# coin-or/Ipopt

Hardware: AMD Instinct MI355X
Metric: KKT factor+solve GFLOP/s (1 numeric LDL^T factorisation + 2 solves per Ipopt iteration) (higher is better)
Workload: dtype f64; 1 GPU; synth_1e6; kkt_dim=1000000, triplet_nnz=20143342, nnz_L=230755000, ordering=nested dissection + minimum-degree leaves (own), supernodes=50052, tree_levels=110, maxfront=3260, num_neg=400000

## Files before the change

ipopt_amd/csrc/device_view.hip.inc:

```
constexpr int FLAG_STRIDE = 32;

typedef double v2d __attribute__((ext_vector_type(2)));
struct DevView {
    const int* sn_colptr; const int* sn_rowptr; const int* sn_rows; const int* rel;
    const int* child_ptr; const int* child_idx; const int* sn_owner; const int* sn_parent; const int* col_owner;
    const long long* panel_off; const long long* cb_off; const long long* minv_off;
    const int* acolptr; const int* apos; const int* arow; const int* acol;
    const int* dup_ptr; const int* dup_src;
    const int* rslot_ptr; const int* rslot_idx; const int* rslot_col; int rslot_len;
    const int* level_sn;
    const FrontMeta* fmeta;
    const int* relinv;
    const GroupLink* gtab;
    const int* tile_tab;
    const ChildMeta* cmeta;
    const int* perm;
    const double* tvals;
    double* aval;
    double* scale;
    double* scale2;
    double* arv;
    unsigned long long* rowmax;
    double* L;
    double* cb;
// ... 18 lines not shown
    unsigned long long* strace;
    const int* chwg_f; const int* chwg_b; const int* chwait; int* sflag_t; int* sflag_dot; double* dpart; v2d* ytag; v2d* xtag;
    int xcd_affine;
    int* apfail;
    int* tcnt;
    double* isg; int* hasis;
    const int* lc_ptr; const LeafLink* lc_link;
    int* sflag_s;
    v2d* cbt; const long long* cbt_off;
    int* sflag_p;
    int* sflag_b; int* sflag_d; int* sepoch;
    int* zpiv;
    int n, nnz_a, nsn, rank;
    int fastpiv;
    double fastu;
    int asm_pull;
    int norestore;
    unsigned long long* dbg;
};

template <int CTRL>
__device__ __forceinline__ double dpp_f64(double x)
{
    int lo = __double2loint(x), hi = __double2hiint(x);
    lo = __builtin_amdgcn_update_dpp(lo, lo, CTRL, 0xF, 0xF, false);
    hi = __builtin_amdgcn_update_dpp(hi, hi, CTRL, 0xF, 0xF, false);
    return __hiloint2double(hi, lo);
}
__device__ __forceinline__ double readlane_f64(double x, int l)
{
// ... 37 lines not shown
```

ipopt_amd/csrc/kernels_big.hip.inc:

```
typedef double v4f64 __attribute__((ext_vector_type(4)));
typedef double double2a __attribute__((ext_vector_type(2), aligned(8)));

__device__ __forceinline__ void big_assemble_column(const DevView& V, const FrontMeta& M, const int fc, const int top_mode)
{
    const int s = M.s, c0 = M.c0, k = M.k, r0 = M.r0, m = M.m; (void)s; (void)c0; (void)r0; (void)k;
    const int lane = threadIdx.x & 63;
    const bool active = fc < m && !(M.asmcut && fc >= M.asmcut);
    double* col = nullptr;
    const bool from_arena = top_mode && V.arena && V.arena_off[s] >= 0;
    const bool skip_owned = top_mode && V.arena;
    if (active) {
        const double* Ar = from_arena ? V.arena + V.arena_off[s] + (size_t)fc * (m - 1) - ((size_t)fc * (fc - 1)) / 2 : nullptr;
        if (fc < k) col = V.L + M.panel_off + (size_t)fc * M.ldp;
        else        col = V.cb + M.cb_off + (size_t)(fc - k) * M.ldt - k;
        if (M.alias) {
            if (from_arena) for (int i = fc + lane; i < m; i += 64) col[i] += Ar[i];
        } else if (V.asm_pull) {
            const double* Cc[4]; const int* Iv[4]; int nc = 0;
            for (int cp = M.ch0; cp < M.ch1 && nc < 4; ++cp) {
                const ChildMeta Cm = V.cmeta[cp];
                if (Cm.aliased || (skip_owned && Cm.owner >= 0) || fc < Cm.rlo || fc > Cm.rhi) continue;
                const int lo = V.relinv[Cm.inv + fc];
                if (lo < 0) continue;
                Cc[nc] = V.cb + Cm.cb_off + (size_t)lo * Cm.ldt; Iv[nc] = V.relinv + Cm.inv; ++nc;
// ... 705 lines not shown
            acc[0][1] = __builtin_amdgcn_mfma_f64_16x16x4f64(a0[u], b1[u], acc[0][1], 0, 0, 0);
            acc[1][0] = __builtin_amdgcn_mfma_f64_16x16x4f64(a1[u], b0[u], acc[1][0], 0, 0, 0);
            acc[1][1] = __builtin_amdgcn_mfma_f64_16x16x4f64(a1[u], b1[u], acc[1][1], 0, 0, 0);
        }
#pragma unroll
    for (int r = 0; r < 2; ++r)
#pragma unroll
        for (int q = 0; q < 2; ++q)
#pragma unroll
            for (int g = 0; g < 4; ++g) {
                const int c = cc0 + r * 16 + l4 + 4 * g, i = i0 + q * 16 + l15;
                if (i < mu && c < climit && i >= c) T[i + (size_t)c * M.ldt] = tv[r][q][g] - acc[r][q][g];
            }
}

__global__ __launch_bounds__(256) void k_big_diag_trsm(DevView V, int list_off, int nrb)
{
    extern __shared__ __attribute__((aligned(16))) char smem_raw[];
    const FrontMeta M = V.fmeta[list_off + blockIdx.x];
    const int role = blockIdx.y;
    const int epoch = V.sepoch[2];
#ifdef MI355X_PIVSTAT
    const bool tprobe = gridDim.x == 1 && threadIdx.x == 0;
    if (tprobe && role == 0) g_dt[0] = wall_clock64();
    if (tprobe && role == 1) g_dt[6] = wall_clock64();
#endif
    if (role == 0) { big_diag_body<4, 256>(V, M, smem_raw, &V.sflag_d[M.s], epoch, nullptr, nullptr, FrontMeta(), 0, 0, V.norestore ? &V.sflag_p[M.s] : nullptr); return; }
    const int tid = threadIdx.x;
    const int s = M.s, k = M.k, m = M.m;
    if (role > nrb) {
        const int t = role - 1 - nrb;
        const int mu = m - k, nt = (mu + 63) >> 6;
        if (M.grem <= 0 || t >= nt * ((M.grem + 63) >> 6)) return;
        if (tid == 0) {
            int spins = 0;
            while (__hip_atomic_load(&V.tcnt[s], __ATOMIC_RELAXED, __HIP_MEMORY_SCOPE_AGENT) < nt) { __builtin_amdgcn_s_sleep(16);
                if (++spins > (1 << 24)) { V.qstat[1] = 1; break; } }
        }
        __syncthreads();
        __builtin_amdgcn_fence(__ATOMIC_ACQUIRE, "agent");
        narrow_tile64(V, M, t);
        return;
// ... 261 lines not shown
        schur_tile_body<64, 64, 256, SCHURQ_LD>(V, M, i0, cc0, mu, 0, 0, As, Bs);
        __syncthreads();
    }
}

__global__ __launch_bounds__(256, 4) void k_big_schur64(DevView V, int list_off, int mode)
{
    int tx = blockIdx.x, fy = blockIdx.y;
    if (V.xcd_affine) xcd_affine(tx, fy);
    const FrontMeta M = V.fmeta[list_off + fy];
    schur64_tile(V, M, tx, mode);
}


constexpr size_t GRP_DB_BYTES = (size_t)64 * 65 * sizeof(double);
__device__ __forceinline__ void grp_fused_body(const DevView& V, const int list_off, const int staged_arg, const int rbw, const int role0)
{
    const int staged = staged_arg;
    extern __shared__ __attribute__((aligned(16))) char smem_raw[];
    const int tid = threadIdx.x, lane = tid & 63, wave = tid >> 6;
    const int l15 = lane & 15, l4 = lane >> 4;
    const FrontMeta M = V.fmeta[list_off + blockIdx.x];
    const int g = M.gpos + 1, role = (int)blockIdx.y + role0;
    const int tail = M.m - M.k;
    int myq = -1, eb0 = 0, nsub = 1;
    if (role < 4) { if (role >= g) return; myq = role; }
    else { eb0 = 64 * rbw * (role - 4); if (eb0 >= tail) return; nsub = min(rbw, (tail - eb0 + 63) >> 6); }
    const int epoch = V.sepoch[2];
#define GSTAMP(i) do { if (V.dbg && blockIdx.x == 0 && role < 4 && tid == 0) V.dbg[32 + 8 * role + (i)] = wall_clock64(); } while (0)
    GSTAMP(0);
// ... 169 lines not shown
    }
    }
    if (myq < 0) return;
    {
        double* Pq = V.L + Gq.panel_off;
        const size_t ldq = (size_t)Gq.ldp;
        const int i = tid & 63, cq = tid >> 6, kq = Gq.k;
        if (!V.norestore) {
#pragma unroll
        for (int e = 0; e < 16; ++e) { const int c = cq + 4 * e; if (i < kq && c < kq && i >= c) Pq[i + (size_t)c * ldq] = Db[i + c * ldb]; }
        }
        FrontMeta Mq = M;
        Mq.s = Gq.s; Mq.c0 = Gq.c0; Mq.k = Gq.k; Mq.m = Gq.m; Mq.panel_off = Gq.panel_off; Mq.ldp = Gq.ldp; Mq.wb = Gq.wb; Mq.minv_off = Gq.minv_off;
        Mq.selfasm = 0; Mq.aq0 = Gq.aq0; Mq.aq1 = Gq.aq1; Mq.bigidx = Gq.bigidx;
        __syncthreads();
        big_diag_body<4, 256, true>(V, Mq, smem_raw, &V.sflag_d[Gq.s], epoch, tsp, crit_Lr, crit_Mp, crit_ibase, myrows, (V.norestore && staged) ? &V.sflag_p[Gq.s] : nullptr);
        if (tsp && tid == 0) { for (int q = 0; q < 28; ++q) V.dbg[64 + q] = tsp[q]; }
        GSTAMP(7);
    }
#undef GSTAMP
}
__global__ __launch_bounds__(256) void k_grp_fused(DevView V, int list_off, int staged, int rbw, int role0) { grp_fused_body(V, list_off, staged, rbw, role0); }
```

ipopt_amd/csrc/kernels_fronts.hip.inc:

```
template <int TS>
__device__ __forceinline__ void publish_col(double* buf, const double (&t)[TS][TS], const int row0, const int jl)
{
#pragma unroll
    for (int b = 0; b < TS; ++b)
        if (jl == b) {
#pragma unroll
            for (int a = 0; a < TS; ++a) { double v = t[a][b]; asm volatile("" : "+v"(v)); buf[row0 + a] = v; }
        }
}

#ifdef MI355X_PIVSTAT
__device__ unsigned long long g_fstat[32];
__device__ unsigned long long g_dt[16], g_dtacc[16];
__device__ unsigned long long g_pivstat[16];
#ifdef MI355X_PIVSTAT_COUNT
#define PIVSTAT(i) do { if (threadIdx.x == 0) atomicAdd(&g_pivstat[i], 1ull); } while (0)
#else
#define PIVSTAT(i) do { } while (0)
#endif
#else
#define PIVSTAT(i) do { } while (0)
#endif

__device__ __forceinline__ double fast_rcp(double d)
// ... 571 lines not shown
                    const int cc = 16 * tc + l15;
#pragma unroll
                    for (int g = 0; g < 4; ++g) { const int rr = 16 * ti + l4 + 4 * g; if (rr < k && cc < k) Lb[rr + cc * ld] -= acc[g]; }
                }
        }
        if (pub) asm volatile("s_waitcnt vmcnt(0)" ::: "memory");
        __syncthreads();
        if (ts) { if (b == 0) ts[18] = clock64(); if (b == 1) ts[21] = clock64(); if (b == 2) ts[24] = clock64(); }
        if (wave == 0) PSTAMP(7);
    }
#undef PSTAMP
    nneg += neg;
    return true;
}

template <int J> __device__ __forceinline__ void fast16_step(double (&a)[16], double (&w)[16], double& rsave, const int l15)
{
    const double t = a[J];
    w[J] = t;
    const double d = bcast16<J>(t);
    const double ri = fast_rcp(d);
    rsave = (l15 == J) ? ri : rsave;
    const double l = t * ri;
    rank1_dpp16<J>(a, t, l);
    a[J] = l;
}
template <int J> __device__ __forceinline__ void fast16_inv(const double (&a)[16], double (&x)[4], const int l15, const int k)
{
    const double m = (l15 > J && l15 < k) ? -a[J] : 0.0;
    subst_dpp16<J>(x[0], m);
// ... 519 lines not shown
        kprev = k; mprev = m; rlp = rl0;
        K0 = K1; K1 = K2;
#pragma unroll
        for (int j = 0; j < 3; ++j) { pos0[j] = pos1[j]; val0[j] = val1[j]; }
        cn0 = cn1; rl0 = rl1;
    }
}

__device__ __forceinline__ void chain_signal(int* flag, const int epoch);
__device__ __forceinline__ void chain_signal_coh(int* flag, const int epoch);
__device__ __forceinline__ void st_coh(double* p, double v);
__device__ __forceinline__ void st_coh(int* p, int v);
__device__ __forceinline__ void st16_coh(double* p, double v0, double v1);
template <int NAP = 2> __device__ __forceinline__ void chain_wait(const int* flag, const int epoch, int* err);
__device__ __forceinline__ void trsm_store_l(const DevView& V, const FrontMeta& M, const double* Lr, const int ibase, const int rlim);
template <int TS, int NT, bool PRE = false>
__device__ __forceinline__ void big_diag_body(const DevView& V, const FrontMeta& M, char* smem_raw, int* flag = nullptr, const int epoch = 0, unsigned long long* ts = nullptr,
                                              const double* late_Lr = nullptr, const FrontMeta& late_M = FrontMeta(), const int late_ibase = 0, const int late_rows = 0, int* pflag = nullptr)
{
    constexpr int G = (NT == 1024) ? 32 : 16, MAXM = G * TS;
    const int tid = threadIdx.x;
    const int s = M.s, c0 = M.c0, k = M.k;
    const int ld = k | 1;
    double* Lb     = reinterpret_cast<double*>(smem_raw);
    double* colbuf = Lb + (size_t)ld * k;
    double* dinv_s = colbuf + 4 * MAXM; double* doff_s = dinv_s + k; double* cm0 = doff_s + k;
    int* ord = reinterpret_cast<int*>(cm0 + k); int* pt_s = ord + k;
    double* P = V.L + M.panel_off;
    const size_t ldp = (size_t)M.ldp;
    int nneg = 0, nzero = 0, ntwo = 0, nsmall = 0, chg = 0;
    DBGSTAMP(0);
// ... 19 lines not shown
#pragma unroll
                    for (int e = 0; e < 2; ++e) { const int q = M.aq0 + tid + e * NT; if (q < M.aq1) { apos_[e] = V.apos[q]; aval_[e] = V.aval[q]; na = e + 1; } }
                }
#pragma unroll
                for (int e = 0; e < 16; ++e) { const int c = cq + 4 * e; if (i < k && c < k && i >= c) { Lb[i + c * ld] = pv[e]; Lb[c + i * ld] = pv[e]; } }
                __syncthreads();
                if (M.selfasm) {
#pragma unroll
                    for (int e = 0; e < 2; ++e) if (e < na) { const int ii = apos_[e] % M.m, cc = apos_[e] / M.m; if (ii < k) { Lb[ii + cc * ld] += aval_[e]; if (ii != cc) Lb[cc + ii * ld] += aval_[e]; } }
                    for (int q = M.aq0 + tid + 2 * NT; q < M.aq1; q += NT) { const int pos = V.apos[q]; const int ii = pos % M.m, cc = pos / M.m; if (ii < k) { const double v = V.aval[q]; Lb[ii + cc * ld] += v; if (ii != cc) Lb[cc + ii * ld] += v; } }
                    __syncthreads();
                }
            }
            DBGT(1);
            if (ts) ts[8] = clock64();
            double cmx;
            {
                const int c = tid >> 2, part = tid & 3;
                double mx = 0.0;
                if (c < k) for (int r = part; r < k; r += 4) mx = fmax(mx, fabs(PRE ? Lb[max(r, c) + min(r, c) * ld] : Lb[r + c * ld]));
                mx = fmax(mx, dpp_f64<0xB1>(mx)); mx = fmax(mx, dpp_f64<0x4E>(mx));
                if (c < k && part == 0) mx = fmax(mx, V.cnorm[c0 + c]); else if (c >= k) mx = 0.0;
                cmx = wave_max_all(mx);
                if ((tid & 63) == 0) colbuf[tid >> 6] = cmx;
                __syncthreads();
                cmx = fmax(fmax(colbuf[0], colbuf[1]), fmax(colbuf[2], colbuf[3]));
            }
            const double zmax = fmax(V.small, ZERO_REL * cmx);
            const double gmax = 1.0 / fmax(fmax(V.pivtol, V.pivtol2), V.fastu);
            DBGT(2);
            if (ts) ts[9] = clock64();
            if (pflag) {
                const PubHook H{P, ldp, V.dinv + c0, V.isg + (size_t)M.bigidx * ISG_STRIDE, pflag, 8 * epoch};
                fast = ldlt_blocked_static(Lb, ld, k, Wp, dinv_s, Isb, shflag, zmax, gmax, nneg, V.dbg, ts, &H);
                if (!fast && tid == 0) __hip_atomic_store(pflag, 8 * epoch + 7, __ATOMIC_RELAXED, __HIP_MEMORY_SCOPE_AGENT);
            } else
            fast = ldlt_blocked_static(Lb, ld, k, Wp, dinv_s, Isb, shflag, zmax, gmax, nneg, V.dbg, ts);
            DBGT(3);
            if (ts) ts[10] = clock64();
            if (fast) {
                DBGSTAMP(1);
#pragma unroll
                for (int e = 0; e < 16; ++e) { const int c = cq + 4 * e; if (i < k && c < k) { const double v = (i > c) ? Lb[i + c * ld] : 0.0; if (flag) st_coh(&P[i + (size_t)c * ldp], v); else P[i + (size_t)c * ldp] = v; if (i <= c) Lb[i + c * ld] = 0.0; } }
                for (int j = tid; j < k; j += NT) { doff_s[j] = 0.0; pt_s[j] = 1; ord[j] = j; }
                {
                    double* Ig = V.isg + (size_t)M.bigidx * ISG_STRIDE;
                    const int nis = ((k + 15) >> 4) * 272;
                    if (flag) { for (int idx = tid; idx < nis; idx += NT) st_coh(&Ig[idx], Isb[idx]); }
                    else for (int idx = tid; idx < nis; idx += NT) Ig[idx] = Isb[idx];
                }
                if (tid == 0) atomicAdd(&V.qstat[3], 1);
                __syncthreads();
// ... 54 lines not shown
#endif
    invert_unit_lower<NT>(Lb, ld, k);
    DBGSTAMP(3);
#ifdef MI355X_PIVSTAT
    if (dprobe) g_dt[4] = wall_clock64();
#endif
    double* Mg = V.minv + M.minv_off;
    for (int idx = tid; idx < k * k; idx += NT) { const int i = idx % k, c = idx / k; Mg[idx] = (i > c) ? Lb[i + c * ld] : (i == c ? 1.0 : 0.0); }
    if (V.dbg && blockIdx.x == 0 && tid == 0) V.dbg[15] = (unsigned long long)k;
}

static size_t diag_lds_bytes(int kk, int maxm)
{
    return (size_t)((kk | 1) * kk + 4 * maxm + 3 * kk) * sizeof(double) + (size_t)(2 * kk + 2) * sizeof(int) + (size_t)(16 * 65 + 4 * 272) * sizeof(double) + 64;
}
template <int TS, int NT = 256>
__global__ __launch_bounds__(NT) void k_big_diag_reg(DevView V, int list_off)
{
    extern __shared__ __attribute__((aligned(16))) char smem_raw[];
    const FrontMeta M = V.fmeta[list_off + blockIdx.x];
    big_diag_body<TS, NT>(V, M, smem_raw);
}

__global__ void k_reduce_stats(const int4* fstat, const int* apfail, const int* owner, int nsn, int rank_filter, int* out)
{
    __shared__ int sh[4][256];
    int a = 0, b = 0, c = 0, d = 0;
    for (int s = blockIdx.x * 256 + threadIdx.x; s < nsn; s += gridDim.x * 256) {
        if (rank_filter >= -1 && owner[s] != rank_filter) continue;
        const int4 v = fstat[s]; a += v.x; b += v.y; c += v.z; d += v.w + apfail[s];
    }
    sh[0][threadIdx.x] = a; sh[1][threadIdx.x] = b; sh[2][threadIdx.x] = c; sh[3][threadIdx.x] = d;
    __syncthreads();
    for (int off = 128; off >= 1; off >>= 1) {
        if (threadIdx.x < off) for (int q = 0; q < 4; ++q) sh[q][threadIdx.x] += sh[q][threadIdx.x + off];
        __syncthreads();
// ... 13 lines not shown
```

ipopt_amd/csrc/numeric.hip:

```cpp
#include <hip/hip_runtime.h>
#include <rccl/rccl.h>
#include <dlfcn.h>
#include <cstdio>
#include <cstring>
#include <cmath>
#include <chrono>
#include <vector>
#include <thread>
#include <map>
#include <string>
#include <algorithm>
#include "numeric.h"
#include "launch_plan.h"
#include "env_knobs.h"
#include "matching_scaling.h"
#include "device_owner.h"
#include "lowrank_host.h"
#include "lbfgs_host.h"

namespace mi355x {

enum KernelKind { KK_GATHER_SCALE = 0, KK_FRONT_WAVE, KK_FRONT_LDS64, KK_FRONT_LDS128, KK_BIG_ASSEMBLE, KK_BIG_DIAG, KK_BIG_TRSM,
                  KK_BIG_SCHUR, KK_STATS, KK_SOLVE_PERM, KK_FWD_WAVE, KK_FWD_LDS, KK_FWD_BIG, KK_BWD_WAVE, KK_BWD_LDS, KK_BWD_BIG, KK_FWD_BIG_UPD, KK_BWD_BIG_DOT, KK_COUNT };
#define DBGSTAMP(slot) do { if (V.dbg && blockIdx.x == 0 && blockIdx.y == 0 && threadIdx.x == 0) { V.dbg[2 * (slot)] = clock64(); V.dbg[2 * (slot) + 1] = wall_clock64(); } } while (0)
// ... 473 lines not shown
                    const long long cap = total + total / 100 + 1024;
                    if (!own_pool.zeroed(&pp, (size_t)cap)) { own_pool.clear(); return false; }
                    kept_pool = pp; kept_pool_doubles = cap;
                } else if (!dalloc(&pp, (size_t)std::max<long long>(end - pool_cut[i], 1))) return false;
                base[i] = (char*)pp;
                in.pool_delta.push_back((long long)((base[i] - base[0]) / (ptrdiff_t)sizeof(double)) - pool_cut[i]);
            }
            V.L = (double*)base[0];
            if (opt.verbose >= 2) fprintf(stderr, "[mi355x_kkt]   pool: %.2f GiB in %zu pieces\n", 8.0 * (double)total / (1024.0 * 1024.0 * 1024.0), pool_cut.size());
        }
        lap("pool");
        knobs = in;
        P = build_launch_plan(Sy, in);
        if (!P.error.empty()) { err_ = P.error; return false; }
        V.fastpiv = in.fastpiv ? 1 : 0; V.asm_pull = in.asm_pull ? 1 : 0; V.fastu = in.fastpiv_floor;
        df_grid_cap = 0;
        if (!P.df_runs.empty()) {
            int per_cu = 0, ncu = 0;
            (void)hipOccupancyMaxActiveBlocksPerMultiprocessor(&per_cu, (const void*)k_front_df, 64, 0);
            (void)hipDeviceGetAttribute(&ncu, hipDeviceAttributeMultiprocessorCount, dev);
            df_grid_cap = std::max(1, per_cu) * std::max(1, ncu);
            if (opt.verbose) { int nl = 0; for (auto& R : P.df_runs) nl += R.nlev; fprintf(stderr, "[mi355x_kkt] small fronts: %d runs covering %d of %d levels in one data-flow launch each (grid <= %d workgroups)\n", (int)P.df_runs.size(), nl, Sy.num_levels, df_grid_cap); }
        }
        lap("host-side schedules and tables");
        if (!upload(P.wgf, &V.chwg_f) || !upload(P.wgb, &V.chwg_b) || !upload(P.chwait, &V.chwait)) return false;
        V.strace = nullptr; V.strace_b = (int)P.wgf.size(); strace_n = 0;
        if (knob_trace("solve") && !P.wgf.empty()) {
            strace_n = 4 * (P.wgf.size() + P.wgb.size());
            if (!dalloc(&V.strace, strace_n)) return false;
            strace_desc.clear();
// ... 30 lines not shown
        if (opt.scaling >= 3 && !d_user_scale) { if (!own_handle.raw(&d_user_scale, Sy.n)) return false; }
        else if (opt.scaling == 2 && !d_user_scale) opt.scaling = 1;
        V.cb = V.L + Sy.l_doubles;
        V.arena = nullptr; V.top_rhs = nullptr; V.rank = opt.rank; V.dbg = nullptr;
        if (knob_trace("clocks")) { if (!dalloc(&V.dbg, 128)) return false; }
        if (multi) { if (!dalloc(&V.arena, (size_t)P.ex.arena_doubles) || !dalloc(&V.top_rhs, (size_t)P.ex.toprhs_doubles)) return false; }
        V.pivtol = opt.pivtol; V.pivtol2 = std::max(opt.pivtol, opt.pivtolmax); V.small = opt.small; V.n = Sy.n; V.nnz_a = Sy.nnz_a; V.nsn = Sy.num_sn; V.xcd_affine = knob_disabled("xcd_affine") ? 0 : 1;
        la_ev.assign(1 + P.grp.size(), LaEvents());
        for (size_t i = 0; i < la_ev.size(); ++i) {
            const std::vector<int>& la2 = i == 0 ? P.la_tiles2 : P.grp[i - 1].la2;
            la_ev[i].A.assign(la2.size(), nullptr); la_ev[i].B.assign(la2.size(), nullptr);
            for (size_t lv = 0; lv < la2.size(); ++lv)
                if (la2[lv] > 0 && (!own_struct.event(&la_ev[i].A[lv], hipEventDisableTiming) || !own_struct.event(&la_ev[i].B[lv], hipEventDisableTiming))) return false;
        }
        HIPCHK(hipFuncSetAttribute((const void*)k_big_diag_reg<4>, hipFuncAttributeMaxDynamicSharedMemorySize, 160 * 1024));
        HIPCHK(hipFuncSetAttribute((const void*)(k_big_diag_reg<4, 1024>), hipFuncAttributeMaxDynamicSharedMemorySize, 160 * 1024));
        HIPCHK(hipFuncSetAttribute((const void*)(k_front_reg<64, 2>), hipFuncAttributeMaxDynamicSharedMemorySize, 160 * 1024));
        HIPCHK(hipFuncSetAttribute((const void*)(k_front_reg<64, 4>), hipFuncAttributeMaxDynamicSharedMemorySize, 160 * 1024));
        HIPCHK(hipFuncSetAttribute((const void*)(k_front_reg<64, 8>), hipFuncAttributeMaxDynamicSharedMemorySize, 160 * 1024));
        HIPCHK(hipFuncSetAttribute((const void*)(k_front_reg<256, 8>), hipFuncAttributeMaxDynamicSharedMemorySize, 160 * 1024));
        HIPCHK(hipFuncSetAttribute((const void*)(k_front_reg<256, 6>), hipFuncAttributeMaxDynamicSharedMemorySize, 160 * 1024));
        HIPCHK(hipFuncSetAttribute((const void*)(k_front_reg<256, 8, true>), hipFuncAttributeMaxDynamicSharedMemorySize, 160 * 1024));
        HIPCHK(hipFuncSetAttribute((const void*)(k_front_reg<256, 6, true, 4>), hipFuncAttributeMaxDynamicSharedMemorySize, 160 * 1024));
        HIPCHK(hipFuncSetAttribute((const void*)k_big_trsm<false>, hipFuncAttributeMaxDynamicSharedMemorySize, 160 * 1024));
        HIPCHK(hipFuncSetAttribute((const void*)k_big_trsm<true>, hipFuncAttributeMaxDynamicSharedMemorySize, 160 * 1024));
        HIPCHK(hipFuncSetAttribute((const void*)k_big_diag_trsm, hipFuncAttributeMaxDynamicSharedMemorySize, 160 * 1024));
        HIPCHK(hipFuncSetAttribute((const void*)k_grp_fused, hipFuncAttributeMaxDynamicSharedMemorySize, 160 * 1024));
        HIPCHK(hipFuncSetAttribute((const void*)k_big_assemble2, hipFuncAttributeMaxDynamicSharedMemorySize, 158 * 1024));
        HIPCHK(hipDeviceSynchronize());
        lap("kernel attributes, zero fills landed");
        ready = true;
        if (keep && comm_kind == 2) make_subcomms();
        return true;
    }

    static size_t trsm_lds(int kk) { return trsm_lds_bytes(kk, false); }
    static int schur_grid(int tiles) { return SCHUR_GM == 2 ? 16 * ((tiles + 7) / 8) : tiles; }
    int grid1d(long long n) const { long long g = (n + 255) / 256; return (int)std::min<long long>(std::max<long long>(g, 1), 2048); }


    bool is_single(const Sched& sc) const { return &sc == &P.single; }
    static int bucket0(const Sched& sc, int lv, int fc) { return sc.base + sc.ptr[(size_t)lv * FC_COUNT + fc]; }
// ... 33 lines not shown
            if (!single) { const bool sm = mm <= 640; return launch_big(lv, b0, sm ? b1 : b0, b1, top_mode, mm, kk, sm ? sc.tiles64[lv] : 0, sm ? 0 : sc.tiles[lv], false); }
            return launch_big(lv, b0, b0 + P.big_split[lv], b1, top_mode, mm, kk, P.part_tiles[0][lv], P.part_tiles[1][lv], true);
        }
        return true;
    }
    bool launch_groups(int lv, int gi) {
        const GrpSched& G = P.grp[gi]; const LaEvents& E = la_ev[1 + gi];
        const int b0 = G.g0[lv], b1 = G.g1[lv], bs = b0 + G.split[lv];
        if (b1 == b0) return true;
        {
            int rbw = 1;
            while (rbw < knobs.grp_rbw_max && (b1 - b0) * (4 + (G.nrb[lv] + rbw - 1) / rbw) > 256) rbw *= 2;
            const int nrbw = (G.nrb[lv] + rbw - 1) / rbw;
            const int st = ((b1 - b0) * (4 + nrbw) <= 256) ? 1 : 0;
            const size_t lds = std::max(diag_lds_bytes(64, 64), GRP_DB_BYTES + trsm_lds_bytes(64, st != 0));
            LAUNCH(KK_BIG_DIAG, k_grp_fused, dim3(b1 - b0, 4 + nrbw), dim3(256), lds, stream, V, b0, st, rbw, 0);
        }
        if (bs > b0 && G.tiles64[lv] > 0) LAUNCH(KK_BIG_SCHUR, k_big_schur64, dim3(G.tiles64[lv], bs - b0), dim3(256), 0, stream, V, b0, 0);
        if (b1 == bs) return true;
        const int nb = b1 - bs;
        if (!la_join()) return false;
        if (G.la2[lv] > 0) {
            if (knobs.p1_small && G.la1[lv] * nb <= 512) {
                LAUNCH(KK_BIG_SCHUR, k_big_schur_p1, dim3(G.p1t[lv], nb), dim3(1024), 0, stream, V, bs);
                if (G.nsplit[lv] < nb) LAUNCH(KK_BIG_SCHUR, k_big_schur, dim3(schur_grid(G.la3[lv]), nb), dim3(SCHUR_NT), 0, stream, V, bs, 4, 0, 0);
            } else LAUNCH(KK_BIG_SCHUR, k_big_schur, dim3(schur_grid(G.la1[lv]), nb), dim3(SCHUR_NT), 0, stream, V, bs, 1, 0, 0);
            return la_fork(E.A[lv], E.B[lv], bs, nb, G.la2[lv]);
        } else if (G.tiles[lv] > 0) LAUNCH(KK_BIG_SCHUR, k_big_schur, dim3(schur_grid(G.tiles[lv]), nb), dim3(SCHUR_NT), 0, stream, V, bs, 0, 0, 0);
        return true;
    }
    std::vector<hipEvent_t> side_evF, side_evJ; bool side_on = !knob_disabled("side_small"); static constexpr int SIDE_MAX_FRONTS = 16;
// ... 16 lines not shown
        for (int q = b0; q < b0 + nfronts && v2; ++q) { v2 = P.asm_fast_ok[q] != 0; maxch = std::max(maxch, (int)P.asm_fast_ok[q]); if (P.asmcut[q]) { ++ncut; cutmax = std::max(cutmax, P.asmcut[q] > 0 ? P.asmcut[q] : 0); } }
        v2 = v2 && (size_t)maxch * ldi * sizeof(int) <= (size_t)158 * 1024 && (nfronts >= 32 && maxch <= 6);
        if (!v2) { LAUNCH(KK_BIG_ASSEMBLE, k_big_assemble, dim3((mm + 3) / 4, nfronts), dim3(256), 0, stream, V, b0, top_mode); return; }
        const int ncols = (ncut == nfronts) ? std::min(mm, cutmax) : mm;
        if (ncols <= 0) return;
        LAUNCH(KK_BIG_ASSEMBLE, k_big_assemble2, dim3((ncols + ASM_CH - 1) / ASM_CH, nfronts), dim3(256), (size_t)maxch * ldi * sizeof(int), stream, V, b0, top_mode, ldi, maxch);
    }
    bool launch_big(int lv, int b0, int bs, int b1, int top_mode, int mm, int kk, int tiles_small, int tiles, bool single) {
        const int nball = b1 - b0;
        if (!(single && P.lv_asm_skip[lv])) launch_assemble(mm, nball, b0, top_mode);
        const int nrb = (mm + 63) / 64;
        if (knobs.fuse_dt && (single || multi) && kk <= 64 && nball * (1 + nrb) <= knobs.fuse_dt_maxwg) {
            const size_t lds = std::max(diag_lds_bytes(kk, 64),
                                        trsm_lds_bytes(kk, true));
            const int ntu = (P.lv_narrow_tiles[lv] > 0 && nball * (1 + nrb + P.lv_narrow_tiles[lv]) <= 256) ? P.lv_narrow_tiles[lv] : 0;
            LAUNCH(KK_BIG_DIAG, k_big_diag_trsm, dim3(nball, 1 + nrb + ntu), dim3(256), lds, stream, V, b0, nrb);
            if (ntu > 0) return true;
            goto updates;
        }
        if (kk <= 64) LAUNCH(KK_BIG_DIAG, k_big_diag_reg<4>, dim3(nball), dim3(256), diag_lds_bytes(kk, 64), stream, V, b0);
        else          LAUNCH(KK_BIG_DIAG, (k_big_diag_reg<4, 1024>), dim3(nball), dim3(1024), diag_lds_bytes(kk, 128), stream, V, b0);
        if (kk <= 64) LAUNCH(KK_BIG_TRSM, k_big_trsm<false>, dim3((mm + 63) / 64, nball), dim3(256), trsm_lds(kk), stream, V, b0, 0);
        else          LAUNCH(KK_BIG_TRSM, k_big_trsm<true>, dim3((mm + 63) / 64, nball), dim3(256), trsm_lds(kk), stream, V, b0, 0);
      updates:
        if (bs > b0 && tiles_small > 0) LAUNCH(KK_BIG_SCHUR, k_big_schur64, dim3(tiles_small, bs - b0), dim3(256), 0, stream, V, b0, 0);
        if (b1 == bs) return true;
        const int nb = b1 - bs;
        b0 = bs;
        if (single && P.la_full[lv] && !la_join()) return false;
        if (single && P.la_tiles2[lv] > 0) {
            LAUNCH(KK_BIG_SCHUR, k_big_schur, dim3(schur_grid(P.la_tiles1[lv]), nb), dim3(SCHUR_NT), 0, stream, V, b0, 1, 0, 0);
            return la_fork(la_ev[0].A[lv], la_ev[0].B[lv], b0, nb, P.la_tiles2[lv]);
        } else if (tiles > 0) LAUNCH(KK_BIG_SCHUR, k_big_schur, dim3(schur_grid(tiles), nb), dim3(SCHUR_NT), 0, stream, V, b0, 0, 0, 0);
        return true;
    }
// ... 1096 lines not shown
```

Before: 9981 GFLOP/s.

## Overlap column-max pivot threshold scan with first diagonal block factorisation

Adds a templated overlap variant of the blocked LDL^T diagonal factorisation. Wave 0 factors the first 16x16 block while the other waves compute the column maxima used for the zero-pivot threshold, and the threshold check on block 0 is deferred until after that. Later blocks split the trailing-tile updates across waves so the next diagonal block factorises alongside them. The aim is to take the serial column-max pass and barrier off the critical path of small-front diagonal kernels. This costs more template instantiations and a reordered rejection check, which could change behaviour at pivot edge cases.

```diff
diff --git a/ipopt_amd/csrc/device_view.hip.inc b/ipopt_amd/csrc/device_view.hip.inc
--- a/ipopt_amd/csrc/device_view.hip.inc
+++ b/ipopt_amd/csrc/device_view.hip.inc
@@ -56,6 +56,7 @@
     int n, nnz_a, nsn, rank;
     int fastpiv;
     double fastu;
+    int piv_overlap;
     int asm_pull;
     int norestore;
     unsigned long long* dbg;
diff --git a/ipopt_amd/csrc/kernels_big.hip.inc b/ipopt_amd/csrc/kernels_big.hip.inc
--- a/ipopt_amd/csrc/kernels_big.hip.inc
+++ b/ipopt_amd/csrc/kernels_big.hip.inc
@@ -743,6 +743,7 @@
             }
 }
 
+template <bool OV>
 __global__ __launch_bounds__(256) void k_big_diag_trsm(DevView V, int list_off, int nrb)
 {
     extern __shared__ __attribute__((aligned(16))) char smem_raw[];
@@ -754,7 +755,7 @@
     if (tprobe && role == 0) g_dt[0] = wall_clock64();
     if (tprobe && role == 1) g_dt[6] = wall_clock64();
 #endif
-    if (role == 0) { big_diag_body<4, 256>(V, M, smem_raw, &V.sflag_d[M.s], epoch, nullptr, nullptr, FrontMeta(), 0, 0, V.norestore ? &V.sflag_p[M.s] : nullptr); return; }
+    if (role == 0) { big_diag_body<4, 256, false, OV>(V, M, smem_raw, &V.sflag_d[M.s], epoch, nullptr, nullptr, FrontMeta(), 0, 0, V.norestore ? &V.sflag_p[M.s] : nullptr); return; }
     const int tid = threadIdx.x;
     const int s = M.s, k = M.k, m = M.m;
     if (role > nrb) {
@@ -1046,6 +1047,7 @@
 
 
 constexpr size_t GRP_DB_BYTES = (size_t)64 * 65 * sizeof(double);
+template <bool OV>
 __device__ __forceinline__ void grp_fused_body(const DevView& V, const int list_off, const int staged_arg, const int rbw, const int role0)
 {
     const int staged = staged_arg;
@@ -1245,10 +1247,11 @@
         Mq.s = Gq.s; Mq.c0 = Gq.c0; Mq.k = Gq.k; Mq.m = Gq.m; Mq.panel_off = Gq.panel_off; Mq.ldp = Gq.ldp; Mq.wb = Gq.wb; Mq.minv_off = Gq.minv_off;
         Mq.selfasm = 0; Mq.aq0 = Gq.aq0; Mq.aq1 = Gq.aq1; Mq.bigidx = Gq.bigidx;
         __syncthreads();
-        big_diag_body<4, 256, true>(V, Mq, smem_raw, &V.sflag_d[Gq.s], epoch, tsp, crit_Lr, crit_Mp, crit_ibase, myrows, (V.norestore && staged) ? &V.sflag_p[Gq.s] : nullptr);
+        big_diag_body<4, 256, true, OV>(V, Mq, smem_raw, &V.sflag_d[Gq.s], epoch, tsp, crit_Lr, crit_Mp, crit_ibase, myrows, (V.norestore && staged) ? &V.sflag_p[Gq.s] : nullptr);
         if (tsp && tid == 0) { for (int q = 0; q < 28; ++q) V.dbg[64 + q] = tsp[q]; }
         GSTAMP(7);
     }
 #undef GSTAMP
 }
-__global__ __launch_bounds__(256) void k_grp_fused(DevView V, int list_off, int staged, int rbw, int role0) { grp_fused_body(V, list_off, staged, rbw, role0); }
+template <bool OV>
+__global__ __launch_bounds__(256) void k_grp_fused(DevView V, int list_off, int staged, int rbw, int role0) { grp_fused_body<OV>(V, list_off, staged, rbw, role0); }
diff --git a/ipopt_amd/csrc/kernels_fronts.hip.inc b/ipopt_amd/csrc/kernels_fronts.hip.inc
--- a/ipopt_amd/csrc/kernels_fronts.hip.inc
+++ b/ipopt_amd/csrc/kernels_fronts.hip.inc
@@ -609,6 +609,160 @@
     return true;
 }
 
+template <bool FIRST>
+__device__ __forceinline__ void ldlt_phase_a(double* Lb, const int ld, const int k, const int b, double* dinv_s, double* Isb, int* rej, const double zmax, const double gmax,
+                                             int& neg, double& rs0, double& mx0, unsigned long long* dbg)
+{
+    const int lane = threadIdx.x & 63, l15 = lane & 15, l4 = lane >> 4;
+    const int c16 = 16 * b, row = c16 + l15;
+#define PSTAMP(i) do { if (FIRST && dbg && blockIdx.x == 0 && blockIdx.y == 0 && lane == 0) dbg[40 + (i)] = clock64(); } while (0)
+    double a[16];
+    double mx = 0.0;
+    PSTAMP(0);
+#pragma unroll
+    for (int c = 0; c < 16; ++c) {
+        const double v = Lb[min(row, k - 1) + min(c16 + c, k - 1) * ld];
+        a[c] = (row < k && c16 + c < k) ? v : ((l15 == c) ? 1.0 : 0.0);
+        if constexpr (FIRST) mx = fmax(mx, (row < k && c16 + c < k && l15 >= c) ? fabs(v) : 0.0);
+    }
+    double rsave = 1.0;
+    asm volatile("s_waitcnt lgkmcnt(0)" ::: "memory"); PSTAMP(1);
+    diag16_step<0>(a, rsave, l15); diag16_step<1>(a, rsave, l15); diag16_step<2>(a, rsave, l15); diag16_step<3>(a, rsave, l15);
+    diag16_step<4>(a, rsave, l15); diag16_step<5>(a, rsave, l15); diag16_step<6>(a, rsave, l15); diag16_step<7>(a, rsave, l15);
+    diag16_step<8>(a, rsave, l15); diag16_step<9>(a, rsave, l15); diag16_step<10>(a, rsave, l15); diag16_step<11>(a, rsave, l15);
+    diag16_step<12>(a, rsave, l15); diag16_step<13>(a, rsave, l15); diag16_step<14>(a, rsave, l15); diag16_step<15>(a, rsave, l15);
+    PSTAMP(2);
+    double gm = 0.0;
+#pragma unroll
+    for (int c = 0; c < 15; ++c) gm = fmax(gm, (l15 > c) ? fabs(a[c]) : 0.0);
+    const bool mine = row < k;
+    bool bad = __ballot(gm > gmax) != 0ull;
+    if constexpr (FIRST) { rs0 = rsave; mx0 = wave_max_all(mx); }
+    else bad |= __ballot(mine && !(fabs(rsave) * zmax < 1.0)) != 0ull;
+    neg += __popcll(__ballot(mine && l4 == 0 && rsave < 0.0));
+    PSTAMP(3);
+    double x[4];
+#pragma unroll
+    for (int q = 0; q < 4; ++q) x[q] = (l15 == 4 * q + l4) ? 1.0 : 0.0;
+    inv16_step<0>(a, x, l15); inv16_step<1>(a, x, l15); inv16_step<2>(a, x, l15); inv16_step<3>(a, x, l15); inv16_step<4>(a, x, l15);
+    inv16_step<5>(a, x, l15); inv16_step<6>(a, x, l15); inv16_step<7>(a, x, l15); inv16_step<8>(a, x, l15); inv16_step<9>(a, x, l15);
+    inv16_step<10>(a, x, l15); inv16_step<11>(a, x, l15); inv16_step<12>(a, x, l15); inv16_step<13>(a, x, l15); inv16_step<14>(a, x, l15);
+    PSTAMP(4);
+    if (dbg && blockIdx.x == 0 && blockIdx.y == 0 && lane == 0) dbg[24 + 2 * b] = clock64();
+    if (bad) { if (lane == 0) rej[0] = 1; }
+    else {
+        if (l4 == 0 && mine) {
+#pragma unroll
+            for (int c = 0; c < 16; ++c) if (c16 + c < k) Lb[row + (c16 + c) * ld] = (l15 > c) ? a[c] : 0.0;
+            dinv_s[row] = rsave;
+        }
+#pragma unroll
+        for (int q = 0; q < 4; ++q) Isb[b * 272 + l15 + (4 * q + l4) * 17] = x[q];
+    }
+    PSTAMP(5);
+#undef PSTAMP
+}
+__device__ __forceinline__ void ldlt_c_tile(double* Lb, const int ld, const int k, const double* Wb, const int c16, const int ti, const int tc, const int l15, const int l4)
+{
+    v4f64_ acc = (v4f64_){0.0, 0.0, 0.0, 0.0};
+    const int ri = 16 * ti + l15;
+#pragma unroll
+    for (int t = 0; t < 4; ++t) {
+        const double al = Lb[min(ri, k - 1) + min(c16 + 4 * t + l4, k - 1) * ld];
+        const double av = (ri < k && c16 + 4 * t + l4 < k) ? al : 0.0;
+        const double bv = Wb[(16 * tc - c16 + l15) + (4 * t + l4) * 65];
+        acc = __builtin_amdgcn_mfma_f64_16x16x4f64(av, bv, acc, 0, 0, 0);
+    }
+    const int cc = 16 * tc + l15;
+#pragma unroll
+    for (int g = 0; g < 4; ++g) { const int rr = 16 * ti + l4 + 4 * g; if (rr < k && cc < k) Lb[rr + cc * ld] -= acc[g]; }
+}
+__device__ __forceinline__ bool ldlt_blocked_overlap(double* Lb, const int ld, const int k, double* Wb, double* dinv_s, double* Isb, int* rej, double* colmax, const double* cnorm,
+                                                     const double small, const double gmax, int& nneg, unsigned long long* dbg, unsigned long long* ts, const bool pub, const PubHook& H)
+{
+    const int tid = threadIdx.x, lane = tid & 63, wave = tid >> 6;
+    const int l15 = lane & 15, l4 = lane >> 4;
+    const int nb = (k + 15) >> 4;
+    if (tid == 0) { rej[0] = 0; rej[1] = 0; }
+    __syncthreads();
+    int neg = 0;
+    double zmax = 0.0, rs0 = 1.0, mx0 = 0.0;
+    if (wave == 0) ldlt_phase_a<true>(Lb, ld, k, 0, dinv_s, Isb, rej, zmax, gmax, neg, rs0, mx0, dbg);
+    else {
+        const int c = lane, part = wave - 1;
+        double mx = 0.0;
+        if (c < k) {
+            for (int r = c + part; r < k; r += 3) if (r >= 16 || c >= 16) mx = fmax(mx, fabs(Lb[r + c * ld]));
+            if (part == 0) mx = fmax(mx, cnorm[c]);
+        }
+        mx = wave_max_all(mx);
+        if (lane == 0) colmax[wave] = mx;
+    }
+    for (int b = 0; b < nb; ++b) {
+        const int c16 = 16 * b;
+        __syncthreads();
+        if (ts) { if (b == 0) ts[16] = clock64(); if (b == 1) ts[19] = clock64(); if (b == 2) ts[22] = clock64(); if (b == 3) ts[25] = clock64(); }
+        if (rej[0]) return false;
+        if (dbg && blockIdx.x == 0 && blockIdx.y == 0 && tid == 0) dbg[25 + 2 * b] = clock64();
+        if (b == 0 && wave == 0) {
+            zmax = fmax(small, ZERO_REL * fmax(fmax(mx0, colmax[1]), fmax(colmax[2], colmax[3])));
+            if (__ballot(l15 < k && !(fabs(rs0) * zmax < 1.0)) != 0ull && lane == 0) rej[1] = 1;
+        }
+        if (b + 1 >= nb) {
+            if (b == 0) { __syncthreads(); if (rej[1]) return false; }
+            if (pub) {
+                publish_subblock(H, Lb, ld, k, dinv_s, Isb, b, tid, (int)blockDim.x);
+                asm volatile("s_waitcnt vmcnt(0)" ::: "memory");
+                __syncthreads();
+                if (tid == 0) __hip_atomic_store(H.pflag, H.fbase + b + 1, __ATOMIC_RELAXED, __HIP_MEMORY_SCOPE_AGENT);
+            }
+            break;
+        }
+        if (pub && wave == 3) publish_subblock(H, Lb, ld, k, dinv_s, Isb, b, lane, 64);
+        for (int t = wave; t < nb - b - 1; t += 4) {
+            const int r = c16 + 16 * (t + 1) + l15;
+            v4f64_ acc = (v4f64_){0.0, 0.0, 0.0, 0.0};
+#pragma unroll
+            for (int u = 0; u < 4; ++u) {
+                const double av = Isb[b * 272 + l15 + (4 * u + l4) * 17];
+                const double bl = Lb[min(r, k - 1) + min(c16 + 4 * u + l4, k - 1) * ld];
+                const double bv = (r < k && c16 + 4 * u + l4 < k) ? bl : 0.0;
+                acc = __builtin_amdgcn_mfma_f64_16x16x4f64(av, bv, acc, 0, 0, 0);
+            }
+            bool big = false;
+#pragma unroll
+            for (int g = 0; g < 4; ++g) {
+                const int c = l4 + 4 * g;
+                const double l = acc[g] * dinv_s[c16 + c];
+                Wb[(r - c16) + c * 65] = acc[g];
+                if (r < k && c16 + c < k) { Lb[r + (c16 + c) * ld] = l; big |= fabs(l) > gmax; }
+            }
+            if (__ballot(big) != 0ull && lane == 0) rej[1] = 1;
+        }
+        __syncthreads();
+        if (ts) { if (b == 0) ts[17] = clock64(); if (b == 1) ts[20] = clock64(); if (b == 2) ts[23] = clock64(); }
+        if (dbg && b == 0 && blockIdx.x == 0 && blockIdx.y == 0 && tid == 0) dbg[46] = clock64();
+        if (rej[1]) return false;
+        if (wave == 0) {
+            ldlt_c_tile(Lb, ld, k, Wb, c16, b + 1, b + 1, l15, l4);
+            if (ts) { if (b == 0) ts[18] = clock64(); if (b == 1) ts[21] = clock64(); if (b == 2) ts[24] = clock64(); }
+            if (dbg && b == 0 && blockIdx.x == 0 && blockIdx.y == 0 && lane == 0) dbg[47] = clock64();
+            ldlt_phase_a<false>(Lb, ld, k, b + 1, dinv_s, Isb, rej, zmax, gmax, neg, rs0, mx0, dbg);
+        } else {
+            int q = 0;
+            for (int tc = b + 1; tc < nb; ++tc)
+                for (int ti = (tc == b + 1) ? tc + 1 : tc; ti < nb; ++ti, ++q)
+                    if (q % 3 == wave - 1) ldlt_c_tile(Lb, ld, k, Wb, c16, ti, tc, l15, l4);
+            if (pub && wave == 3) {
+                asm volatile("s_waitcnt vmcnt(0)" ::: "memory");
+                if (lane == 0) __hip_atomic_store(H.pflag, H.fbase + b + 1, __ATOMIC_RELAXED, __HIP_MEMORY_SCOPE_AGENT);
+            }
+        }
+    }
+    nneg += neg;
+    return true;
+}
+
 template <int J> __device__ __forceinline__ void fast16_step(double (&a)[16], double (&w)[16], double& rsave, const int l15)
 {
     const double t = a[J];
@@ -1158,7 +1312,7 @@
 __device__ __forceinline__ void st16_coh(double* p, double v0, double v1);
 template <int NAP = 2> __device__ __forceinline__ void chain_wait(const int* flag, const int epoch, int* err);
 __device__ __forceinline__ void trsm_store_l(const DevView& V, const FrontMeta& M, const double* Lr, const int ibase, const int rlim);
-template <int TS, int NT, bool PRE = false>
+template <int TS, int NT, bool PRE = false, bool OV = false>
 __device__ __forceinline__ void big_diag_body(const DevView& V, const FrontMeta& M, char* smem_raw, int* flag = nullptr, const int epoch = 0, unsigned long long* ts = nullptr,
                                               const double* late_Lr = nullptr, const FrontMeta& late_M = FrontMeta(), const int late_ibase = 0, const int late_rows = 0, int* pflag = nullptr)
 {
@@ -1208,28 +1362,36 @@
             }
             DBGT(1);
             if (ts) ts[8] = clock64();
-            double cmx;
-            {
-                const int c = tid >> 2, part = tid & 3;
-                double mx = 0.0;
-                if (c < k) for (int r = part; r < k; r += 4) mx = fmax(mx, fabs(PRE ? Lb[max(r, c) + min(r, c) * ld] : Lb[r + c * ld]));
-                mx = fmax(mx, dpp_f64<0xB1>(mx)); mx = fmax(mx, dpp_f64<0x4E>(mx));
-                if (c < k && part == 0) mx = fmax(mx, V.cnorm[c0 + c]); else if (c >= k) mx = 0.0;
-                cmx = wave_max_all(mx);
-                if ((tid & 63) == 0) colbuf[tid >> 6] = cmx;
-                __syncthreads();
-                cmx = fmax(fmax(colbuf[0], colbuf[1]), fmax(colbuf[2], colbuf[3]));
-            }
-            const double zmax = fmax(V.small, ZERO_REL * cmx);
             const double gmax = 1.0 / fmax(fmax(V.pivtol, V.pivtol2), V.fastu);
-            DBGT(2);
-            if (ts) ts[9] = clock64();
-            if (pflag) {
+            if constexpr (OV) {
+                DBGT(2);
+                if (ts) ts[9] = clock64();
                 const PubHook H{P, ldp, V.dinv + c0, V.isg + (size_t)M.bigidx * ISG_STRIDE, pflag, 8 * epoch};
-                fast = ldlt_blocked_static(Lb, ld, k, Wp, dinv_s, Isb, shflag, zmax, gmax, nneg, V.dbg, ts, &H);
-                if (!fast && tid == 0) __hip_atomic_store(pflag, 8 * epoch + 7, __ATOMIC_RELAXED, __HIP_MEMORY_SCOPE_AGENT);
-            } else
-            fast = ldlt_blocked_static(Lb, ld, k, Wp, dinv_s, Isb, shflag, zmax, gmax, nneg, V.dbg, ts);
+                fast = ldlt_blocked_overlap(Lb, ld, k, Wp, dinv_s, Isb, shflag, colbuf, V.cnorm + c0, V.small, gmax, nneg, V.dbg, ts, pflag != nullptr, H);
+                if (pflag && !fast && tid == 0) __hip_atomic_store(pflag, 8 * epoch + 7, __ATOMIC_RELAXED, __HIP_MEMORY_SCOPE_AGENT);
+            } else {
+                double cmx;
+                {
+                    const int c = tid >> 2, part = tid & 3;
+                    double mx = 0.0;
+                    if (c < k) for (int r = part; r < k; r += 4) mx = fmax(mx, fabs(PRE ? Lb[max(r, c) + min(r, c) * ld] : Lb[r + c * ld]));
+                    mx = fmax(mx, dpp_f64<0xB1>(mx)); mx = fmax(mx, dpp_f64<0x4E>(mx));
+                    if (c < k && part == 0) mx = fmax(mx, V.cnorm[c0 + c]); else if (c >= k) mx = 0.0;
+                    cmx = wave_max_all(mx);
+                    if ((tid & 63) == 0) colbuf[tid >> 6] = cmx;
+                    __syncthreads();
+                    cmx = fmax(fmax(colbuf[0], colbuf[1]), fmax(colbuf[2], colbuf[3]));
+                }
+                const double zmax = fmax(V.small, ZERO_REL * cmx);
+                DBGT(2);
+                if (ts) ts[9] = clock64();
+                if (pflag) {
+                    const PubHook H{P, ldp, V.dinv + c0, V.isg + (size_t)M.bigidx * ISG_STRIDE, pflag, 8 * epoch};
+                    fast = ldlt_blocked_static(Lb, ld, k, Wp, dinv_s, Isb, shflag, zmax, gmax, nneg, V.dbg, ts, &H);
+                    if (!fast && tid == 0) __hip_atomic_store(pflag, 8 * epoch + 7, __ATOMIC_RELAXED, __HIP_MEMORY_SCOPE_AGENT);
+                } else
+                fast = ldlt_blocked_static(Lb, ld, k, Wp, dinv_s, Isb, shflag, zmax, gmax, nneg, V.dbg, ts);
+            }
             DBGT(3);
             if (ts) ts[10] = clock64();
             if (fast) {
@@ -1314,12 +1476,12 @@
 {
     return (size_t)((kk | 1) * kk + 4 * maxm + 3 * kk) * sizeof(double) + (size_t)(2 * kk + 2) * sizeof(int) + (size_t)(16 * 65 + 4 * 272) * sizeof(double) + 64;
 }
-template <int TS, int NT = 256>
+template <int TS, int NT = 256, bool OV = false>
 __global__ __launch_bounds__(NT) void k_big_diag_reg(DevView V, int list_off)
 {
     extern __shared__ __attribute__((aligned(16))) char smem_raw[];
     const FrontMeta M = V.fmeta[list_off + blockIdx.x];
-    big_diag_body<TS, NT>(V, M, smem_raw);
+    big_diag_body<TS, NT, false, OV>(V, M, smem_raw);
 }
 
 __global__ void k_reduce_stats(const int4* fstat, const int* apfail, const int* owner, int nsn, int rank_filter, int* out)
diff --git a/ipopt_amd/csrc/numeric.hip b/ipopt_amd/csrc/numeric.hip
--- a/ipopt_amd/csrc/numeric.hip
+++ b/ipopt_amd/csrc/numeric.hip
@@ -511,6 +511,7 @@
         P = build_launch_plan(Sy, in);
         if (!P.error.empty()) { err_ = P.error; return false; }
         V.fastpiv = in.fastpiv ? 1 : 0; V.asm_pull = in.asm_pull ? 1 : 0; V.fastu = in.fastpiv_floor;
+        V.piv_overlap = knob_disabled("piv_overlap") ? 0 : 1;
         df_grid_cap = 0;
         if (!P.df_runs.empty()) {
             int per_cu = 0, ncu = 0;
@@ -571,6 +572,7 @@
                 if (la2[lv] > 0 && (!own_struct.event(&la_ev[i].A[lv], hipEventDisableTiming) || !own_struct.event(&la_ev[i].B[lv], hipEventDisableTiming))) return false;
         }
         HIPCHK(hipFuncSetAttribute((const void*)k_big_diag_reg<4>, hipFuncAttributeMaxDynamicSharedMemorySize, 160 * 1024));
+        HIPCHK(hipFuncSetAttribute((const void*)(k_big_diag_reg<4, 256, true>), hipFuncAttributeMaxDynamicSharedMemorySize, 160 * 1024));
         HIPCHK(hipFuncSetAttribute((const void*)(k_big_diag_reg<4, 1024>), hipFuncAttributeMaxDynamicSharedMemorySize, 160 * 1024));
         HIPCHK(hipFuncSetAttribute((const void*)(k_front_reg<64, 2>), hipFuncAttributeMaxDynamicSharedMemorySize, 160 * 1024));
         HIPCHK(hipFuncSetAttribute((const void*)(k_front_reg<64, 4>), hipFuncAttributeMaxDynamicSharedMemorySize, 160 * 1024));
@@ -581,8 +583,10 @@
         HIPCHK(hipFuncSetAttribute((const void*)(k_front_reg<256, 6, true, 4>), hipFuncAttributeMaxDynamicSharedMemorySize, 160 * 1024));
         HIPCHK(hipFuncSetAttribute((const void*)k_big_trsm<false>, hipFuncAttributeMaxDynamicSharedMemorySize, 160 * 1024));
         HIPCHK(hipFuncSetAttribute((const void*)k_big_trsm<true>, hipFuncAttributeMaxDynamicSharedMemorySize, 160 * 1024));
-        HIPCHK(hipFuncSetAttribute((const void*)k_big_diag_trsm, hipFuncAttributeMaxDynamicSharedMemorySize, 160 * 1024));
-        HIPCHK(hipFuncSetAttribute((const void*)k_grp_fused, hipFuncAttributeMaxDynamicSharedMemorySize, 160 * 1024));
+        HIPCHK(hipFuncSetAttribute((const void*)k_big_diag_trsm<false>, hipFuncAttributeMaxDynamicSharedMemorySize, 160 * 1024));
+        HIPCHK(hipFuncSetAttribute((const void*)k_big_diag_trsm<true>, hipFuncAttributeMaxDynamicSharedMemorySize, 160 * 1024));
+        HIPCHK(hipFuncSetAttribute((const void*)k_grp_fused<false>, hipFuncAttributeMaxDynamicSharedMemorySize, 160 * 1024));
+        HIPCHK(hipFuncSetAttribute((const void*)k_grp_fused<true>, hipFuncAttributeMaxDynamicSharedMemorySize, 160 * 1024));
         HIPCHK(hipFuncSetAttribute((const void*)k_big_assemble2, hipFuncAttributeMaxDynamicSharedMemorySize, 158 * 1024));
         HIPCHK(hipDeviceSynchronize());
         lap("kernel attributes, zero fills landed");
@@ -646,7 +650,8 @@
             const int nrbw = (G.nrb[lv] + rbw - 1) / rbw;
             const int st = ((b1 - b0) * (4 + nrbw) <= 256) ? 1 : 0;
             const size_t lds = std::max(diag_lds_bytes(64, 64), GRP_DB_BYTES + trsm_lds_bytes(64, st != 0));
-            LAUNCH(KK_BIG_DIAG, k_grp_fused, dim3(b1 - b0, 4 + nrbw), dim3(256), lds, stream, V, b0, st, rbw, 0);
+            if (V.piv_overlap) LAUNCH(KK_BIG_DIAG, k_grp_fused<true>, dim3(b1 - b0, 4 + nrbw), dim3(256), lds, stream, V, b0, st, rbw, 0);
+            else               LAUNCH(KK_BIG_DIAG, k_grp_fused<false>, dim3(b1 - b0, 4 + nrbw), dim3(256), lds, stream, V, b0, st, rbw, 0);
         }
         if (bs > b0 && G.tiles64[lv] > 0) LAUNCH(KK_BIG_SCHUR, k_big_schur64, dim3(G.tiles64[lv], bs - b0), dim3(256), 0, stream, V, b0, 0);
         if (b1 == bs) return true;
@@ -693,11 +698,13 @@
             const size_t lds = std::max(diag_lds_bytes(kk, 64),
                                         trsm_lds_bytes(kk, true));
             const int ntu = (P.lv_narrow_tiles[lv] > 0 && nball * (1 + nrb + P.lv_narrow_tiles[lv]) <= 256) ? P.lv_narrow_tiles[lv] : 0;
-            LAUNCH(KK_BIG_DIAG, k_big_diag_trsm, dim3(nball, 1 + nrb + ntu), dim3(256), lds, stream, V, b0, nrb);
+            if (V.piv_overlap) LAUNCH(KK_BIG_DIAG, k_big_diag_trsm<true>, dim3(nball, 1 + nrb + ntu), dim3(256), lds, stream, V, b0, nrb);
+            else               LAUNCH(KK_BIG_DIAG, k_big_diag_trsm<false>, dim3(nball, 1 + nrb + ntu), dim3(256), lds, stream, V, b0, nrb);
             if (ntu > 0) return true;
             goto updates;
         }
-        if (kk <= 64) LAUNCH(KK_BIG_DIAG, k_big_diag_reg<4>, dim3(nball), dim3(256), diag_lds_bytes(kk, 64), stream, V, b0);
+        if (kk <= 64 && V.piv_overlap) LAUNCH(KK_BIG_DIAG, (k_big_diag_reg<4, 256, true>), dim3(nball), dim3(256), diag_lds_bytes(kk, 64), stream, V, b0);
+        else if (kk <= 64) LAUNCH(KK_BIG_DIAG, k_big_diag_reg<4>, dim3(nball), dim3(256), diag_lds_bytes(kk, 64), stream, V, b0);
         else          LAUNCH(KK_BIG_DIAG, (k_big_diag_reg<4, 1024>), dim3(nball), dim3(1024), diag_lds_bytes(kk, 128), stream, V, b0);
         if (kk <= 64) LAUNCH(KK_BIG_TRSM, k_big_trsm<false>, dim3((mm + 63) / 64, nball), dim3(256), trsm_lds(kk), stream, V, b0, 0);
         else          LAUNCH(KK_BIG_TRSM, k_big_trsm<true>, dim3((mm + 63) / 64, nball), dim3(256), trsm_lds(kk), stream, V, b0, 0);
```

Measured after the change: 10050 GFLOP/s, median of 6. About the same (+0.7%).
